# SiTronXD/vk3dGaussianSplatting

Hardware: AMD Instinct MI355X
Metric: Msplats/s + total frame ms (InitSortList/RadixSort/FindRanges/Render split) (higher is better)
Workload: dtype f32; 1 GPU; Garden-30k shape: 5,834,784 gaussians @ 1920x1080; num_gaussians=5834784, width=1920, height=1080, render_mode=exact, render_kernel=auto, sort_algorithm=radix4, frames_in_flight=1, parallelism=single GPU

## Files before the change

### vk3dgaussiansplatting_amd/csrc/gs_project.hip

```cpp
#include <cstdlib>
#include "gs_splat_math.h"
#include "gs_sort_words.h"

namespace gs {

__device__ __forceinline__ Mat3 mat3_mul(const Mat3& a, const Mat3& b) {
    Mat3 c;
#pragma unroll
    for (int j = 0; j < 3; ++j)
#pragma unroll
        for (int i = 0; i < 3; ++i) {
            float acc = a.m[0][i] * b.m[j][0];
            acc = acc + a.m[1][i] * b.m[j][1];
            acc = acc + a.m[2][i] * b.m[j][2];
            c.m[j][i] = acc;
        }
    return c;
}
__device__ __forceinline__ Mat3 mat3_transpose(const Mat3& a) {
    Mat3 t;
#pragma unroll
    for (int j = 0; j < 3; ++j)
#pragma unroll
        for (int i = 0; i < 3; ++i) t.m[j][i] = a.m[i][j];
// ... 284 lines not shown

    if (g < n && !wave_skip) {
        const float px = scene.pos[g], py = scene.pos[(size_t)n + g], pz = scene.pos[2 * (size_t)n + g];
        float vp[4];
        mat4_mul_vec4(fp.view, px, py, pz, 1.0f, vp);
        if (!(-vp[2] <= fp.near_plane)) {
            float q[4];
            mat4_mul_vec4(fp.proj, vp[0], vp[1], vp[2], vp[3], q);
            const float ndc_x = q[0] / q[3];
            const float ndc_y = q[1] / q[3];
            if (!(fabsf(ndc_x) > fp.ndc_cull || fabsf(ndc_y) > fp.ndc_cull)) {
                float nd = (-vp[2] - fp.near_plane) / (fp.far_plane - fp.near_plane);
                nd = clampf(nd, 0.0f, 1.0f);
                const uint32_t depth_key = f2u_sat(nd * 4294967296.0f);
                bool band_skip = false;

                if (band) {
                    const float hgt = (float)fp.height;
                    const float tfx = fp.tan_fov_y * (float)fp.width / hgt;
                    const float tx = clampf(vp[0] / vp[2], -tfx * fp.in_view_limit, tfx * fp.in_view_limit);
                    const float ty = clampf(vp[1] / vp[2], -fp.tan_fov_y * fp.in_view_limit, fp.tan_fov_y * fp.in_view_limit);
                    const float rmax = radius_bound(fp, tx, ty, vp[2], scene.sig2[g]);
                    const float sy_b = (1.0f - ndc_y) * 0.5f * hgt;
                    band_skip = misses_owned_rows(fp, sy_b - rmax, sy_b + rmax);
                }
                if (!band_skip) {
                    float scale[3], rot[4], cov[3], cov0[3];
#pragma unroll
                    for (int a = 0; a < 3; ++a) scale[a] = scene.scale[a * (size_t)n + g];
#pragma unroll
                    for (int a = 0; a < 4; ++a) rot[a] = scene.rot[a * (size_t)n + g];
                    get_covariance(fp, scale, rot, vp, cov, cov0);

                    float sx, sy;
                    screen_position(fp, ndc_x, ndc_y, sx, sy);

                    const float det = cov[0] * cov[2] - cov[1] * cov[1];
                    const float radius = tile_extent_radius(cov[0], cov[1], cov[2]);
                    const int gw = (int)fp.grid_w, gh = (int)fp.grid_h;
                    const int min_x = clampi(f2i_sat((sx - radius) / 16.0f), 0, gw);
                    const int min_y = clampi(f2i_sat((sy - radius) / 16.0f), 0, gh);
                    int tx = f2i_sat((sx + radius) / 16.0f);
                    int ty = f2i_sat((sy + radius) / 16.0f);
                    const int max_x = clampi(tx == 2147483647 ? tx : tx + 1, 0, gw);
                    const int max_y = clampi(ty == 2147483647 ? ty : ty + 1, 0, gh);

                    int y0 = min_y > (int)fp.row_begin ? min_y : (int)fp.row_begin;
                    int y1 = max_y < (int)fp.row_end ? max_y : (int)fp.row_end;
                    if (y1 < y0) y1 = y0;
                    const int k0 = owned_rows_below(fp, y0), k1 = owned_rows_below(fp, y1);
                    count = (uint32_t)(max_x - min_x) * (uint32_t)(k1 - k0);

                    kept = true;
                    rec0 = make_float4(sx, sy, 0.0f, 0.0f);
                    rec2 = make_float4(0.0f, cov[0], cov[1], cov[2]);
                    if (count != 0u) {
                        float opacity = scene.opacity[g];
                        float inv_x = 0.0f, inv_y = 0.0f, inv_z = 0.0f;
                        if (det != 0.0f) {
                            const float det_inv = 1.0f / det;
                            inv_x = cov[2] * det_inv;
                            inv_y = -cov[1] * det_inv;
                            inv_z = cov[0] * det_inv;
                            if constexpr (AA) {
                                const float det0 = cov0[0] * cov0[2] - cov0[1] * cov0[1];
                                const float r = det0 / det;
                                opacity = opacity * sqrtf(r > kAntialiasFloor ? (r < 1.0f ? r : 1.0f) : kAntialiasFloor);
                            }
                        } else {
                            opacity = 0.0f;
                        }
                        rec0.z = inv_x; rec0.w = inv_y;
                        rec2.x = opacity;
                        if constexpr (VIEW_Z) {
                            sc.view_z[g] = -vp[2];
                            sc.depth_key[g] = depth_key;
                            sc.extents[g] = make_uint2((uint32_t)min_x | ((uint32_t)k0 << 16), (uint32_t)max_x | ((uint32_t)k1 << 16));
                        }
                        float res[3];
                        splat_colour<NT_SH, SH_K>(fp, scene.sh + g, n, px, py, pz, res);
                        rec1 = make_float4(inv_z, res[0], res[1], res[2]);
                        if constexpr (!VIEW_Z) sc.depth_key[g] = depth_key;
#if GS_EMIT_PASS0
                        count |= (depth_key & (uint32_t)(kBins - 1)) << 28;
#endif
                        if constexpr (!VIEW_Z) sc.extents[g] = make_uint2((uint32_t)min_x | ((uint32_t)k0 << 16),
                                                                          (uint32_t)max_x | ((uint32_t)k1 << 16));
                    }
                }
            }
        }
#if GS_EMIT_PASS0
        sc.tiles_touched[g] = count & 0x0FFFFFFFu;
#else
        sc.tiles_touched[g] = count;
#endif
    } else if (g < n) {
        sc.tiles_touched[g] = 0u;
    }

#if GS_EMIT_PASS0
    const uint32_t digit = count >> 28;
    count &= 0x0FFFFFFFu;
#endif
    s_raster[threadIdx.x * 3 + 0] = rec0;
    s_raster[threadIdx.x * 3 + 1] = rec1;
    s_raster[threadIdx.x * 3 + 2] = rec2;
    const uint32_t wsum = wave_sum_to_lane63(count);
    const uint64_t emits = __ballot(count != 0u);
    const uint32_t wflags = (uint32_t)__popcll(emits);
    const bool wave_kept = __ballot(kept) != 0ull;
#if GS_EMIT_PASS0
    __shared__ uint32_t s_hist[kProjThreads / 64][kBins];
    if (lane_id() < kBins) s_hist[wave_id()][lane_id()] = 0u;
    __builtin_amdgcn_wave_barrier();
    for (uint64_t todo = emits; todo != 0ull;) {
        const uint32_t d = (uint32_t)__builtin_amdgcn_readlane((int)digit, (int)__builtin_ctzll(todo));
        const bool mine = count != 0u && digit == d;
        const uint32_t dsum = wave_sum_to_lane63(mine ? count : 0u);
        if (lane_id() == 63) s_hist[wave_id()][d] = dsum;
        todo &= ~__ballot(mine);
    }
#endif
    if (lane_id() == 63) {
        s_wave_sum[wave_id()] = wsum;
        s_wave_flags[wave_id()] = wflags;
#ifndef GS_PROJECT_WRITE_ALL
#define GS_PROJECT_WRITE_ALL 0
#endif
#ifndef GS_PROJECT_WRITE_KEPT
#define GS_PROJECT_WRITE_KEPT 0
#endif
#ifndef GS_PROJECT_RECORD_CHUNK
#define GS_PROJECT_RECORD_CHUNK 16
#endif
        static_assert(GS_PROJECT_RECORD_CHUNK == 16 || GS_PROJECT_RECORD_CHUNK == 64, "a quarter wave or a wave");
        uint32_t wrote;
        if (band) wrote = wsum != 0u ? 0xFu : 0u;
        else if (GS_PROJECT_WRITE_ALL || GS_PROJECT_WRITE_KEPT) wrote = (GS_PROJECT_WRITE_ALL || wave_kept) ? 0xFu : 0u;
        else if (GS_PROJECT_RECORD_CHUNK == 64) wrote = emits != 0ull ? 0xFu : 0u;
        else wrote = ((emits & 0xFFFFull) ? 1u : 0u) | ((emits & 0xFFFF0000ull) ? 2u : 0u) |
                     ((emits & 0xFFFF00000000ull) ? 4u : 0u) | ((emits >> 48) ? 8u : 0u);
        s_wave_emits[wave_id()] = wrote;
        sc.wave_wrote[blk * (kProjThreads / 64) + wave_id()] = (uint8_t)wrote;
    }
    __syncthreads();
    {
        const uint32_t first = blk * kProjThreads;
        const uint32_t valid = (n - first) < (uint32_t)kProjThreads ? (n - first) : (uint32_t)kProjThreads;
        float4* out = reinterpret_cast<float4*>(sc.raster + first);
#pragma unroll
        for (int q = 0; q < 3; ++q) {
            const uint32_t i = q * kProjThreads + threadIdx.x;
            if (i < valid * 3u && ((s_wave_emits[i / 192u] >> ((i / 48u) & 3u)) & 1u)) out[i] = s_raster[i];
        }
    }
    uint32_t t = 0;
#pragma unroll
    for (int w = 0; w < kProjThreads / 64; ++w) t += s_wave_sum[w];
    if (threadIdx.x == 0) {
        sc.block_sums[blk] = t;
        if (fp.splat_first) sc.block_flags[blk] = s_wave_flags[0] + s_wave_flags[1] + s_wave_flags[2] + s_wave_flags[3];
    }
#if GS_EMIT_PASS0
    if (threadIdx.x < kBins) {
        const uint32_t v = (s_hist[0][threadIdx.x] + s_hist[1][threadIdx.x]) + (s_hist[2][threadIdx.x] + s_hist[3][threadIdx.x]);
        const uint32_t nb = (n + (uint32_t)kProjThreads - 1u) / (uint32_t)kProjThreads;
        uint32_t* hist = pass0_hist_of(sc.block_sums, nb);
        uint32_t* chunk = pass0_chunk_of(sc.block_sums, nb);
        hist[(size_t)blk * kBins + threadIdx.x] = v;
        if (v != 0u)
            (void)__hip_atomic_fetch_add(&chunk[((size_t)fp.parity * pass0_chunks(nb) + blk / kPass0Chunk) * kBins + threadIdx.x],
                                         v, __ATOMIC_RELAXED, __HIP_MEMORY_SCOPE_AGENT);
    }
#endif
    if (!fp.splat_first) register_emit_helpers(fp, sc, blk, t);
}

struct ScanJob { const uint32_t* sums; uint32_t* offsets; SortParams* params; uint32_t capacity;
                 uint32_t* host_note;
                 SortParams* done_params; };
constexpr uint32_t kScanClearWgs = 8;
struct Pass0Scan { const uint32_t* hist; uint32_t* offs; const uint32_t* chunk_in; uint4* chunk_zero; uint32_t chunks; };

__device__ __forceinline__ void scan_pass0_chunk(const Pass0Scan& p0, uint32_t c, uint32_t num_blocks) {
    __shared__ uint32_t s_part[16][kBins], s_rows[16][kBins];
    const uint32_t tid = threadIdx.x, lane = tid & 63u, wave = tid >> 6, d = tid & 15u;
    const uint32_t row = c * kPass0Chunk + (tid >> 4);
    const uint32_t v = row < num_blocks ? p0.hist[(size_t)row * kBins + d] : 0u;
    uint32_t before = 0u;
    for (uint32_t k = tid >> 4; k < c; k += 64u) before += p0.chunk_in[(size_t)k * kBins + d];
    before += (uint32_t)__shfl_xor((int)before, 16, 64);
    before += (uint32_t)__shfl_xor((int)before, 32, 64);
    uint32_t inc = v;
    uint32_t up = (uint32_t)__shfl_up((int)inc, 16, 64);
    inc += lane >= 16u ? up : 0u;
    up = (uint32_t)__shfl_up((int)inc, 32, 64);
    inc += lane >= 32u ? up : 0u;
    if (lane < (uint32_t)kBins) s_part[wave][d] = before;
    if (lane >= 48u) s_rows[wave][d] = inc;
    __syncthreads();
    uint32_t base = 0u;
#pragma unroll
    for (uint32_t w = 0; w < 16u; ++w) base += s_part[w][d] + (w < wave ? s_rows[w][d] : 0u);
    if (row <= num_blocks) p0.offs[(size_t)row * kBins + d] = base + inc - v;
}

__global__ __launch_bounds__(1024) void k_scan_blocks(const ScanJob job0, const ScanJob job1, uint32_t jobs, uint32_t num_blocks,
                                                       uint4* __restrict__ zero_a, uint32_t n16_a,
                                                       uint4* __restrict__ zero_b, uint32_t n16_b,
                                                       uint32_t* __restrict__ next_help_count, const Pass0Scan p0) {
    if (blockIdx.x >= jobs + kScanClearWgs) {
        scan_pass0_chunk(p0, blockIdx.x - jobs - kScanClearWgs, num_blocks);
        return;
    }
    if (blockIdx.x >= jobs) {
        const uint32_t k = blockIdx.x - jobs;
        if (k == 0u && threadIdx.x == 0 && next_help_count) { next_help_count[0] = 0u; next_help_count[2] = 0u; }
        for (uint32_t i = k * 1024u + threadIdx.x; i < n16_a; i += kScanClearWgs * 1024u) zero_a[i] = make_uint4(0u, 0u, 0u, 0u);
        for (uint32_t i = k * 1024u + threadIdx.x; i < n16_b; i += kScanClearWgs * 1024u) zero_b[i] = make_uint4(0u, 0u, 0u, 0u);
        for (uint32_t i = k * 1024u + threadIdx.x; i < p0.chunks * 4u; i += kScanClearWgs * 1024u) p0.chunk_zero[i] = make_uint4(0u, 0u, 0u, 0u);
        return;
    }
    const ScanJob job = blockIdx.x == 0 ? job0 : job1;
    const uint32_t* __restrict__ block_sums = job.sums;
    uint32_t* __restrict__ block_offsets = job.offsets;
    SortParams* params = job.params;
    const uint32_t capacity = job.capacity;
    __shared__ uint64_t s_wave_tot[16];
    const int tid = threadIdx.x, lane = tid & 63, wave = tid >> 6;
    const uint32_t per = (((num_blocks + 1023u) / 1024u) + 3u) & ~3u;
    const uint4* in4 = reinterpret_cast<const uint4*>(block_sums + (size_t)tid * per);
    uint4* out4 = reinterpret_cast<uint4*>(block_offsets + (size_t)tid * per);
    auto sat = [](uint64_t x) { return (uint32_t)(x > 0xFFFFFFFFull ? 0xFFFFFFFFull : x); };
    constexpr uint32_t kHeld = 8;
    const bool held = per / 4 <= kHeld;
    uint4 v[kHeld];
    uint64_t sum = 0;
    if (held) {
#pragma unroll
        for (uint32_t i = 0; i < kHeld; ++i) v[i] = i < per / 4 ? in4[i] : make_uint4(0u, 0u, 0u, 0u);
#pragma unroll
        for (uint32_t i = 0; i < kHeld; ++i) sum += (uint64_t)v[i].x + v[i].y + v[i].z + v[i].w;
    } else {
#pragma unroll 4
        for (uint32_t i = 0; i < per / 4; ++i) {
            const uint4 w = in4[i];
            sum += (uint64_t)w.x + w.y + w.z + w.w;
        }
    }
    const uint64_t inc = wave_inclusive_scan64(sum);
    if (lane == 63) s_wave_tot[wave] = inc;
    __syncthreads();
    uint64_t run = inc - sum;
    for (int w = 0; w < wave; ++w) run += s_wave_tot[w];
    if (tid == 1023) {
        const uint64_t counter = run + sum;
        const uint32_t e = counter < capacity ? (uint32_t)counter : capacity;
        params->counter = counter;
        params->num_elems = e;
        params->num_groups = (e + kSortTile - 1) / kSortTile;
        params->groups_per_seg = (params->num_groups + kSegments - 1) / kSegments;
        params->overflow = counter > capacity ? 1u : 0u;
        if (job.done_params) {
            const bool redo = counter > capacity;
            job.done_params->counter = counter;
            job.done_params->num_elems = redo ? e : 0u;
            job.done_params->num_groups = redo ? params->num_groups : 0u;
            job.done_params->groups_per_seg = redo ? params->groups_per_seg : 0u;
            job.done_params->overflow = redo ? 1u : 0u;
        }
        if (job.host_note) __hip_atomic_store(job.host_note, e + 1u, __ATOMIC_RELAXED, __HIP_MEMORY_SCOPE_SYSTEM);
    }
    if (held) {
#pragma unroll
        for (uint32_t i = 0; i < kHeld; ++i) {
            uint4 o;
            o.x = sat(run); run += v[i].x;
            o.y = sat(run); run += v[i].y;
            o.z = sat(run); run += v[i].z;
            o.w = sat(run); run += v[i].w;
            if (i < per / 4) out4[i] = o;
        }
    } else {
#pragma unroll 4
        for (uint32_t i = 0; i < per / 4; ++i) {
            const uint4 w = in4[i];
            uint4 o;
            o.x = sat(run); run += w.x;
            o.y = sat(run); run += w.y;
            o.z = sat(run); run += w.z;
            o.w = sat(run); run += w.w;
            out4[i] = o;
        }
    }
}

constexpr int kEmitChunk = 4 * kProjThreads;
static_assert(kEmitSlice % kEmitChunk == 0, "a slice is a whole number of rounds");

#ifndef GS_EMIT_XCD_ORDER
#define GS_EMIT_XCD_ORDER 0
#endif
template <bool SORTED, bool P0 = false>
__global__ __launch_bounds__(kProjThreads) void k_emit(const FrameParams fp, const SplatScratch sc,
                                                        uint32_t* __restrict__ out_lo,
                                                        uint32_t* __restrict__ out_hi,
                                                        uint32_t* __restrict__ out_id, uint32_t num_blocks,
                                                        uint32_t helpers, const uint32_t* __restrict__ sorted_ids,
                                                        const uint32_t* __restrict__ sorted_counts,
                                                        uint32_t* __restrict__ p0_lo = nullptr, uint32_t* __restrict__ p0_hi = nullptr,
                                                        uint32_t* __restrict__ p0_id = nullptr, const SortParams* __restrict__ done = nullptr) {
    static_assert(!(SORTED && P0), "the splat-first list is in depth order already");
    const uint32_t* __restrict__ sums = SORTED ? sc.sorted_sums : sc.block_sums;
    __shared__ __attribute__((aligned(16))) uint32_t s_dig[P0 ? kBins : 1][kProjThreads / 64];
    __shared__ uint32_t s_gofs[P0 ? kBins : 1];
    __shared__ uint32_t s_tot[P0 ? kBins : 1];
    __shared__ uint8_t s_idx[P0 ? kProjThreads : 1];
    __shared__ uint32_t s_incl[kProjThreads];
    __shared__ uint32_t s_wave_tot[kProjThreads / 64];
    __shared__ uint2 s_ext[kProjThreads];
    __shared__ uint32_t s_depth[kProjThreads];
    __shared__ uint32_t s_owner[kEmitChunk];
    __shared__ uint32_t s_wmax[kProjThreads / 64];
    const uint32_t n = SORTED ? sc.aux_params[0].num_elems : fp.num_gaussians;
    const int tid = threadIdx.x;
    uint32_t blk = blockIdx.x - helpers, slice = 0u;
    if (blockIdx.x < helpers) {
        const uint32_t h = blockIdx.x;
        if (h >= sc.help_count[fp.parity]) return;
        const uint2 rec = sc.help_list[h];
        blk = rec.x; slice = rec.y;
        if (blk >= num_blocks || slice == 0u) return;
        const uint32_t first = sc.help_slot[blk];
        if (first == kEmitNoHelp || h - first + 1u != slice) return;
        const uint32_t t = sums[blk];
        if (t <= kEmitSlice || slice > (t - 1u) / kEmitSlice) return;
    } else if constexpr (P0 && GS_EMIT_XCD_ORDER != 0) {
        blk = xcd_group(blk, (num_blocks + 7u) / 8u);
        if (blk >= num_blocks) return;
    }
    const uint32_t g = blk * kProjThreads + tid;
    const uint32_t total = sums[blk];
    if (!owns_every_row(fp) && total == 0) return;
    const uint32_t base = sc.block_offsets[blk];
    const bool alone = slice == 0u && total > kEmitSlice && sc.help_slot[blk] == kEmitNoHelp;
    uint32_t cnt = 0u, my_depth = 0u;
    uint2 my_ext = make_uint2(0u, 0u);
    if (g < n) {
        if constexpr (SORTED) {
            my_depth = sorted_ids[g];
            cnt = fp.hi16 ? (uint32_t)reinterpret_cast<const uint16_t*>(sorted_counts)[g] : sorted_counts[g];
            my_ext = sc.extents[my_depth];
        } else {
            cnt = sc.tiles_touched[g];
            my_ext = sc.extents[g];
            my_depth = sc.depth_key[g];
        }
    }
    bool fused = false;
    uint32_t my_offs = 0u, dstart16 = 0u;
    if constexpr (P0) {
        fused = done->overflow == 0u;
        if (tid < kBins) {
            my_offs = sc.pass0_offs[(size_t)blk * kBins + tid];
            s_tot[tid] = sc.pass0_offs[(size_t)num_blocks * kBins + tid];
        }
    }
    if (total == 0) return;
    if (base >= fp.capacity) return;
    if (P0 && fused) {
        const uint32_t dg = cnt != 0u ? my_depth & (uint32_t)(kBins - 1) : 0u;
        uint32_t m_lo = 0xFFFFFFFFu, m_hi = 0xFFFFFFFFu;
#pragma unroll
        for (int b = 0; b < kRadixBits; ++b) {
            const int32_t sbit = __builtin_amdgcn_sbfe((int32_t)dg, (uint32_t)b, 1u);
            const uint64_t bal = __ballot(sbit != 0);
            m_lo &= ~((uint32_t)bal ^ (uint32_t)sbit);
            m_hi &= ~((uint32_t)(bal >> 32) ^ (uint32_t)sbit);
        }
        const uint64_t same = ((uint64_t)m_hi << 32) | m_lo;
        const uint32_t in_wave = mbcnt(same);
        if (lane_id() < kBins) s_dig[lane_id()][wave_id()] = 0u;
        __builtin_amdgcn_wave_barrier();
        if (in_wave == 0u) s_dig[dg][wave_id()] = (uint32_t)__popcll(same);
        __syncthreads();
        static_assert(kProjThreads / 64 == 4, "one 16-byte LDS read per digit");
        const uint4 c = *reinterpret_cast<const uint4*>(&s_dig[lane_id() & 15][0]);
        const uint32_t tot = c.x + c.y + c.z + c.w;
        dstart16 = row16_inclusive_scan(tot) - tot;
        const uint32_t wb = dstart16 + (wave_id() > 0 ? c.x : 0u) + (wave_id() > 1 ? c.y : 0u) + (wave_id() > 2 ? c.z : 0u);
        const uint32_t slot = (uint32_t)__shfl((int)wb, (int)dg, 64) + in_wave;
        if ((uint32_t)__shfl((int)tot, (int)dg, 64) == (uint32_t)kProjThreads) {
            s_ext[tid] = my_ext;
            s_depth[tid] = my_depth;
            s_idx[tid] = (uint8_t)tid;
        } else {
            s_incl[slot] = cnt;
            s_ext[slot] = my_ext;
            s_depth[slot] = my_depth;
            s_idx[slot] = (uint8_t)tid;
            __syncthreads();
            cnt = s_incl[tid];
        }
    } else {
        s_ext[tid] = my_ext;
        s_depth[tid] = my_depth;
        if constexpr (P0) s_idx[tid] = (uint8_t)tid;
    }
    const uint32_t inc = wave_inclusive_scan(cnt);
    if (lane_id() == 63) s_wave_tot[wave_id()] = inc;
    __syncthreads();
    uint32_t wbase = 0;
    for (int w = 0; w < wave_id(); ++w) wbase += s_wave_tot[w];
    s_incl[tid] = wbase + inc;
    __syncthreads();
    if constexpr (P0) {
        if (tid < kBins) {
            uint32_t gofs = base;
            if (fused) {
                uint32_t smaller = 0u;
                for (int d = 0; d < tid; ++d) smaller += s_tot[d];
                gofs = smaller + my_offs - (dstart16 > 0u ? s_incl[dstart16 - 1u] : 0u);
            }
            s_gofs[tid] = gofs;
        }
        if (fused) { out_lo = p0_lo; out_hi = p0_hi; out_id = p0_id; }
    }

    const uint32_t g0 = blk * kProjThreads;
    const uint32_t my_excl = s_incl[tid] - cnt;
    const uint32_t c_begin = slice * kEmitSlice;
    const uint32_t c_end = alone || total - c_begin < kEmitSlice ? total : c_begin + kEmitSlice;
    for (uint32_t c0 = c_begin; c0 < c_end; c0 += kEmitChunk) {
#pragma unroll
        for (int k = 0; k < kEmitChunk / kProjThreads; ++k) s_owner[k * kProjThreads + tid] = 0u;
        __syncthreads();
        if (cnt != 0u) {
            if (my_excl >= c0) {
                if (my_excl - c0 < (uint32_t)kEmitChunk) s_owner[my_excl - c0] = (uint32_t)tid + 1u;
            } else if (my_excl + cnt > c0) {
                s_owner[0] = (uint32_t)tid + 1u;
            }
        }
        __syncthreads();
        uint4 o = *reinterpret_cast<const uint4*>(&s_owner[4 * tid]);
        o.y = o.y > o.x ? o.y : o.x;
        o.z = o.z > o.y ? o.z : o.y;
        o.w = o.w > o.z ? o.w : o.z;
        const uint32_t winc = wave_inclusive_max(o.w);
        if (lane_id() == 63) s_wmax[wave_id()] = winc;
        uint32_t prev = __shfl_up(winc, 1, 64);
        if (lane_id() == 0) prev = 0u;
        __syncthreads();
        for (int w = 0; w < wave_id(); ++w) prev = prev > s_wmax[w] ? prev : s_wmax[w];
        o.x = o.x > prev ? o.x : prev;
        o.y = o.y > prev ? o.y : prev;
        o.z = o.z > prev ? o.z : prev;
        o.w = o.w > prev ? o.w : prev;
        *reinterpret_cast<uint4*>(&s_owner[4 * tid]) = o;
        __syncthreads();
#pragma unroll
        for (int k = 0; k < kEmitChunk / kProjThreads; ++k) {
            const uint32_t jj = (uint32_t)(k * kProjThreads + tid);
            const uint32_t j = c0 + jj;
            if (j < total) {
                const uint32_t s = s_owner[jj] - 1u;
                const uint32_t excl = s > 0u ? s_incl[s - 1u] : 0u;
                const uint32_t id_local = j - excl;
                const uint2 ext = s_ext[s];
                const uint32_t min_x = ext.x & 0xFFFFu, y0 = ext.x >> 16, max_x = ext.y & 0xFFFFu;
                const uint32_t wdt = max_x - min_x;
                uint32_t ry = (uint32_t)((float)id_local * __builtin_amdgcn_rcpf((float)wdt));
                int32_t rx = (int32_t)(id_local - ry * wdt);
                if (rx < 0) { --ry; rx += (int32_t)wdt; }
                else if ((uint32_t)rx >= wdt) { ++ry; rx -= (int32_t)wdt; }
                const uint32_t tile_key = (y0 + ry) * fp.grid_w + (min_x + (uint32_t)rx);
                const uint64_t out = P0 ? (uint64_t)(s_gofs[s_depth[s] & (uint32_t)(kBins - 1)] + j) : (uint64_t)base + j;
                const uint32_t id = g0 + (P0 ? (uint32_t)s_idx[s] : s);
                if (out < fp.capacity) {
                    if (!SORTED && fp.packed) {
                        out_lo[out] = s_depth[s];
                        out_id[out] = (tile_key << 16) | (id & 0xFFFFu);
                        reinterpret_cast<uint8_t*>(out_hi)[out] = (uint8_t)(id >> 16);
                    } else {
                        if (fp.hi16) reinterpret_cast<uint16_t*>(out_hi)[out] = (uint16_t)tile_key;
                        else out_hi[out] = tile_key;
                        if constexpr (SORTED) out_id[out] = s_depth[s];
                        else { out_lo[out] = s_depth[s]; out_id[out] = id; }
                    }
                }
            }
        }
        __syncthreads();
    }
}

template <int SH_K, bool AA>
static void launch_project_cut(const FrameParams& fp, const SceneBuffers& scene, const SplatScratch& sc, uint32_t blocks, bool nt_sh,
                               hipStream_t stream) {
    if (sc.view_z) {
        if (nt_sh) hipLaunchKernelGGL((k_project<true, true, SH_K, AA>), dim3(blocks), dim3(kProjThreads), 0, stream, fp, scene, sc, blocks);
        else hipLaunchKernelGGL((k_project<false, true, SH_K, AA>), dim3(blocks), dim3(kProjThreads), 0, stream, fp, scene, sc, blocks);
    } else {
        if (nt_sh) hipLaunchKernelGGL((k_project<true, false, SH_K, AA>), dim3(blocks), dim3(kProjThreads), 0, stream, fp, scene, sc, blocks);
        else hipLaunchKernelGGL((k_project<false, false, SH_K, AA>), dim3(blocks), dim3(kProjThreads), 0, stream, fp, scene, sc, blocks);
    }
}

void launch_project(const FrameParams& fp, const SceneBuffers& scene, const SplatScratch& sc,
                    hipStream_t stream) {
    const uint32_t blocks = (fp.num_gaussians + kProjThreads - 1) / kProjThreads;
    if (blocks == 0) return;
    const bool listed = !(fp.row_begin == 0u && fp.row_end == fp.grid_h) && fp.row_stride == 1u;
    if (listed) hipLaunchKernelGGL(k_band_cull, dim3((blocks * 4u + (uint32_t)kCullThreads - 1u) / (uint32_t)kCullThreads), dim3(kCullThreads), 0, stream,
                                   fp, scene, sc, blocks);
#ifndef GS_PROJECT_NT_SH_ABOVE
#define GS_PROJECT_NT_SH_ABOVE ((size_t)256u << 20)
#endif
    const bool nt_sh = (size_t)fp.num_gaussians * 236u > GS_PROJECT_NT_SH_ABOVE;
    const int cut = sh_cut_of_mode(fp.sh_mode);
    if (fp.antialias) {
        switch (cut) {
            case 4: launch_project_cut<4, true>(fp, scene, sc, blocks, nt_sh, stream); break;
            case 9: launch_project_cut<9, true>(fp, scene, sc, blocks, nt_sh, stream); break;
            default: launch_project_cut<0, true>(fp, scene, sc, blocks, nt_sh, stream); break;
        }
    } else {
        switch (cut) {
            case 4: launch_project_cut<4, false>(fp, scene, sc, blocks, nt_sh, stream); break;
            case 9: launch_project_cut<9, false>(fp, scene, sc, blocks, nt_sh, stream); break;
            default: launch_project_cut<0, false>(fp, scene, sc, blocks, nt_sh, stream); break;
        }
    }
}

template <int SH_K>
__global__ __launch_bounds__(256) void k_debug_colour(const FrameParams fp, const SceneBuffers scene, const float4* records, float4* out) {
    const uint32_t n = fp.num_gaussians;
    const uint32_t g = blockIdx.x * 256u + threadIdx.x;
    if (g >= n) return;
    float4 o = make_float4(0.f, 0.f, 0.f, 0.f);
    if (records[2 * (size_t)g].w != 0.0f) {
        float res[3];
        splat_colour<false, SH_K>(fp, scene.sh + g, n, scene.pos[g], scene.pos[(size_t)n + g], scene.pos[2 * (size_t)n + g], res);
        o = make_float4(res[0], res[1], res[2], 1.0f);
    }
    out[g] = o;
}

void launch_debug_colour(const FrameParams& fp, const SceneBuffers& scene, const float* records, float* out_rgba, hipStream_t stream) {
    const uint32_t blocks = (fp.num_gaussians + 255u) / 256u;
    if (!blocks) return;
    float4* out = reinterpret_cast<float4*>(out_rgba);
    const float4* recs = reinterpret_cast<const float4*>(records);
    switch (sh_cut_of_mode(fp.sh_mode)) {
        case 4: hipLaunchKernelGGL(k_debug_colour<4>, dim3(blocks), dim3(256), 0, stream, fp, scene, recs, out); break;
        case 9: hipLaunchKernelGGL(k_debug_colour<9>, dim3(blocks), dim3(256), 0, stream, fp, scene, recs, out); break;
        default: hipLaunchKernelGGL(k_debug_colour<0>, dim3(blocks), dim3(256), 0, stream, fp, scene, recs, out); break;
    }
}

__global__ __launch_bounds__(256) void k_debug_records(const FrameParams fp, const SceneBuffers scene, const SplatScratch sc, float4* out) {
    const uint32_t n = fp.num_gaussians;
    const uint32_t g = blockIdx.x * 256u + threadIdx.x;
    if (g >= n) return;
    float4 o0 = make_float4(0.f, 0.f, 0.f, 0.f), o1 = o0;
    if (sc.tiles_touched[g] == 0u) {
        float vp[4];
        mat4_mul_vec4(fp.view, scene.pos[g], scene.pos[(size_t)n + g], scene.pos[2 * (size_t)n + g], 1.0f, vp);
        if (!(-vp[2] <= fp.near_plane)) {
            float q[4];
            mat4_mul_vec4(fp.proj, vp[0], vp[1], vp[2], vp[3], q);
            const float ndc_x = q[0] / q[3];
            const float ndc_y = q[1] / q[3];
            if (!(fabsf(ndc_x) > fp.ndc_cull || fabsf(ndc_y) > fp.ndc_cull)) {
                float scale[3], rot[4], cov[3], cov0[3];
#pragma unroll
                for (int a = 0; a < 3; ++a) scale[a] = scene.scale[a * (size_t)n + g];
#pragma unroll
                for (int a = 0; a < 4; ++a) rot[a] = scene.rot[a * (size_t)n + g];
                get_covariance(fp, scale, rot, vp, cov, cov0);
                float sx, sy;
                screen_position(fp, ndc_x, ndc_y, sx, sy);
                o0 = make_float4(sx, sy, 0.0f, 1.0f);
                o1 = make_float4(0.0f, cov[0], cov[1], cov[2]);
            }
        }
    }
    out[2 * (size_t)g] = o0;
    out[2 * (size_t)g + 1] = o1;
}

void launch_debug_records(const FrameParams& fp, const SceneBuffers& scene, const SplatScratch& sc, float* out_records, hipStream_t stream) {
    const uint32_t blocks = (fp.num_gaussians + 255u) / 256u;
    if (!blocks) return;
    hipLaunchKernelGGL(k_debug_records, dim3(blocks), dim3(256), 0, stream, fp, scene, sc, reinterpret_cast<float4*>(out_records));
}

void launch_scan_blocks(const FrameParams& fp, const SplatScratch& sc, SortParams* params,
                        uint32_t* ranges, uint32_t* coarse, hipStream_t stream) {
    const uint32_t blocks = (fp.num_gaussians + kProjThreads - 1) / kProjThreads;
    const uint32_t n16_ranges = (fp.grid_w * fp.grid_h * 2u + 3u) / 4u;
    const uint32_t n16_coarse = (uint32_t)(kMaxSortPasses * kBins * kCoarse) / 4u;
    const ScanJob elements{sc.block_sums, sc.block_offsets, params, fp.capacity, sc.elems_note, GS_EMIT_PASS0 ? params + 1 : nullptr};
    const ScanJob splats{sc.block_flags, sc.flag_offsets, sc.aux_params, fp.num_gaussians, nullptr, nullptr};
    const uint32_t jobs = fp.splat_first ? 2u : 1u;
    const uint32_t chunks = GS_EMIT_PASS0 ? pass0_chunks(blocks) : 0u;
    const size_t half = (size_t)chunks * kBins;
    const Pass0Scan p0{sc.pass0_hist, sc.pass0_offs, sc.pass0_chunk + fp.parity * half,
                       reinterpret_cast<uint4*>(sc.pass0_chunk + (fp.parity ^ 1u) * half), chunks};
    hipLaunchKernelGGL(k_scan_blocks, dim3(jobs + kScanClearWgs + chunks), dim3(1024), 0, stream, elements, splats, jobs, blocks,
                       reinterpret_cast<uint4*>(ranges), n16_ranges, reinterpret_cast<uint4*>(coarse), n16_coarse,
                       sc.help_count + (fp.parity ^ 1u), p0);
}

void launch_emit(const FrameParams& fp, const SplatScratch& sc, const SortBuffers& sb, bool pass0,
                 hipStream_t stream) {
    const uint32_t blocks = (fp.num_gaussians + kProjThreads - 1) / kProjThreads;
    if (blocks == 0) return;
    const uint32_t helpers = emit_helpers(fp.capacity);
    if (pass0) {
        const uint32_t owners = GS_EMIT_XCD_ORDER != 0 ? 8u * ((blocks + 7u) / 8u) : blocks;
        hipLaunchKernelGGL((k_emit<false, true>), dim3(helpers + owners), dim3(kProjThreads), 0, stream, fp, sc, sb.lo[0],
                           sb.hi[0], sb.id[0], blocks, helpers, (const uint32_t*)nullptr, (const uint32_t*)nullptr,
                           sb.lo[1], sb.hi[1], sb.id[1], (const SortParams*)(sb.params + 1));
        return;
    }
    hipLaunchKernelGGL((k_emit<false>), dim3(helpers + blocks), dim3(kProjThreads), 0, stream, fp, sc, sb.lo[0],
                       sb.hi[0], sb.id[0], blocks, helpers, (const uint32_t*)nullptr, (const uint32_t*)nullptr);
}

__global__ __launch_bounds__(kProjThreads) void k_splat_list(const FrameParams fp, const SplatScratch sc,
                                                              uint32_t* __restrict__ out_depth, uint32_t* __restrict__ out_count,
                                                              uint32_t* __restrict__ out_id) {
    __shared__ uint32_t s_cnt[kProjThreads / 64], s_flag[kProjThreads / 64];
    const uint32_t blk = blockIdx.x, g = blk * kProjThreads + threadIdx.x;
    if (blk == 0u && threadIdx.x == 0u) sc.help_count[fp.parity] = 0u;
    if (sc.block_sums[blk] == 0u) return;
    const uint32_t cnt = g < fp.num_gaussians ? sc.tiles_touched[g] : 0u;
    const uint32_t dk = cnt != 0u ? sc.depth_key[g] : 0u;
    const uint64_t off0 = sc.block_offsets[blk];
    const uint32_t fpos0 = sc.flag_offsets[blk];
    const uint32_t inc = wave_inclusive_scan(cnt);
    const uint64_t fb = __ballot(cnt != 0u);
    if (lane_id() == 63) { s_cnt[wave_id()] = inc; s_flag[wave_id()] = (uint32_t)__popcll(fb); }
    __syncthreads();
    uint64_t off = off0 + (inc - cnt);
    uint32_t pos = fpos0 + (uint32_t)__popcll(fb & ((1ull << lane_id()) - 1ull));
    for (int w = 0; w < wave_id(); ++w) { off += s_cnt[w]; pos += s_flag[w]; }
    if (cnt != 0u) {
        const uint64_t room = off < fp.capacity ? (uint64_t)fp.capacity - off : 0ull;
        const uint32_t kept = room < cnt ? (uint32_t)room : cnt;
        out_depth[pos] = dk;
        if (fp.hi16) reinterpret_cast<uint16_t*>(out_count)[pos] = (uint16_t)kept;
        else out_count[pos] = kept;
        out_id[pos] = g;
    }
}

constexpr int kSumsBlocksPerWg = 8;
__global__ __launch_bounds__(kProjThreads) void k_sorted_sums(const FrameParams fp, const SplatScratch sc,
                                                               const uint32_t* __restrict__ sorted_counts, uint32_t num_blocks) {
    const uint32_t ve = sc.aux_params[0].num_elems;
    const int lane = lane_id();
#pragma unroll
    for (int it = 0; it < kSumsBlocksPerWg / (kProjThreads / 64); ++it) {
        const uint32_t blk = blockIdx.x * kSumsBlocksPerWg + (uint32_t)(it * (kProjThreads / 64) + wave_id());
        if (blk >= num_blocks) return;
        const uint32_t i0 = blk * kProjThreads + 4u * (uint32_t)lane;
        uint32_t c[4] = {0u, 0u, 0u, 0u};
        if (i0 + 3u < ve) {
            if (fp.hi16) {
                const uint2 v = *reinterpret_cast<const uint2*>(reinterpret_cast<const uint16_t*>(sorted_counts) + i0);
                c[0] = v.x & 0xFFFFu; c[1] = v.x >> 16; c[2] = v.y & 0xFFFFu; c[3] = v.y >> 16;
            } else {
                const uint4 v = *reinterpret_cast<const uint4*>(sorted_counts + i0);
                c[0] = v.x; c[1] = v.y; c[2] = v.z; c[3] = v.w;
            }
        } else {
#pragma unroll
            for (int k = 0; k < 4; ++k)
                if (i0 + k < ve) c[k] = fp.hi16 ? (uint32_t)reinterpret_cast<const uint16_t*>(sorted_counts)[i0 + k] : sorted_counts[i0 + k];
        }
        const uint32_t t = (uint32_t)__builtin_amdgcn_readlane((int)wave_sum_to_lane63(c[0] + c[1] + c[2] + c[3]), 63);
        if (lane == 0) sc.sorted_sums[blk] = t;
        if (t > kEmitSlice) {
            const uint32_t extra = (t - 1u) / kEmitSlice;
            uint32_t slot = 0u;
            if (lane == 0) {
                slot = atomicAdd(&sc.help_count[fp.parity], extra);
                if ((uint64_t)slot + extra > (uint64_t)emit_helpers(fp.capacity)) slot = kEmitNoHelp;
                sc.help_slot[blk] = slot;
            }
            slot = (uint32_t)__builtin_amdgcn_readfirstlane((int)slot);
            if (slot != kEmitNoHelp)
                for (uint32_t i = (uint32_t)lane; i < extra; i += 64u) sc.help_list[slot + i] = make_uint2(blk, i + 1u);
        }
    }
}

void launch_splat_list(const FrameParams& fp, const SplatScratch& sc, const SortBuffers& sb, hipStream_t stream) {
    const uint32_t blocks = (fp.num_gaussians + kProjThreads - 1) / kProjThreads;
    if (blocks == 0) return;
    hipLaunchKernelGGL(k_splat_list, dim3(blocks), dim3(kProjThreads), 0, stream, fp, sc, sb.lo[1], sb.hi[1], sb.id[1]);
}

void launch_gather_sorted(const FrameParams& fp, const SplatScratch& sc, const SortBuffers& sb, int sorted, hipStream_t stream) {
    const uint32_t blocks = (fp.num_gaussians + kProjThreads - 1) / kProjThreads;
    if (blocks == 0) return;
    hipLaunchKernelGGL(k_sorted_sums, dim3((blocks + kSumsBlocksPerWg - 1) / kSumsBlocksPerWg), dim3(kProjThreads), 0, stream, fp, sc,
                       (const uint32_t*)sb.hi[sorted], blocks);
    const ScanJob sorted_blocks{sc.sorted_sums, sc.block_offsets, sc.aux_params + 1, fp.capacity};
    hipLaunchKernelGGL(k_scan_blocks, dim3(1), dim3(1024), 0, stream, sorted_blocks, sorted_blocks, 1u, blocks,
                       (uint4*)nullptr, 0u, (uint4*)nullptr, 0u, (uint32_t*)nullptr, Pass0Scan{});
}

void launch_emit_sorted(const FrameParams& fp, const SplatScratch& sc, const SortBuffers& sb, int sorted, hipStream_t stream) {
    const uint32_t blocks = (fp.num_gaussians + kProjThreads - 1) / kProjThreads;
    if (blocks == 0) return;
    const uint32_t helpers = emit_helpers(fp.capacity);
    hipLaunchKernelGGL((k_emit<true>), dim3(helpers + blocks), dim3(kProjThreads), 0, stream, fp, sc, (uint32_t*)nullptr,
                       sb.hi[0], sb.id[0], blocks, helpers, (const uint32_t*)sb.id[sorted], (const uint32_t*)sb.hi[sorted]);
}

}
```

Baseline: 6613 Msplats/s.

## Add slot-record emit path for fused pass0 with per-splat records in LDS

Adds a dedicated emit kernel body for the fused pass-0 path. It packs each splat's count, extents, index and depth into one LDS record, pre-sorts splats within the block by low depth digit, and computes owners with a vectorized max-scan. Each output element then does a single LDS record read instead of several scattered arrays, and the next block's loads are prefetched when a workgroup handles multiple blocks. The aim is fewer LDS accesses and barriers in the emit stage, at the cost of more code, more LDS use, and extra ballot and scan work per block.

```diff
diff --git a/vk3dgaussiansplatting_amd/csrc/gs_project.hip b/vk3dgaussiansplatting_amd/csrc/gs_project.hip
--- a/vk3dgaussiansplatting_amd/csrc/gs_project.hip
+++ b/vk3dgaussiansplatting_amd/csrc/gs_project.hip
@@ -610,15 +610,15 @@
 #ifndef GS_EMIT_XCD_ORDER
 #define GS_EMIT_XCD_ORDER 0
 #endif
-template <bool SORTED, bool P0 = false>
-__global__ __launch_bounds__(kProjThreads) void k_emit(const FrameParams fp, const SplatScratch sc,
-                                                        uint32_t* __restrict__ out_lo,
-                                                        uint32_t* __restrict__ out_hi,
-                                                        uint32_t* __restrict__ out_id, uint32_t num_blocks,
-                                                        uint32_t helpers, const uint32_t* __restrict__ sorted_ids,
-                                                        const uint32_t* __restrict__ sorted_counts,
-                                                        uint32_t* __restrict__ p0_lo = nullptr, uint32_t* __restrict__ p0_hi = nullptr,
-                                                        uint32_t* __restrict__ p0_id = nullptr, const SortParams* __restrict__ done = nullptr) {
+template <bool SORTED, bool P0>
+__device__ __forceinline__ void emit_walk(const FrameParams& fp, const SplatScratch& sc,
+                                          uint32_t* __restrict__ out_lo,
+                                          uint32_t* __restrict__ out_hi,
+                                          uint32_t* __restrict__ out_id, uint32_t num_blocks,
+                                          uint32_t helpers, const uint32_t* __restrict__ sorted_ids,
+                                          const uint32_t* __restrict__ sorted_counts,
+                                          uint32_t* __restrict__ p0_lo, uint32_t* __restrict__ p0_hi,
+                                          uint32_t* __restrict__ p0_id, const SortParams* __restrict__ done) {
     static_assert(!(SORTED && P0), "the splat-first list is in depth order already");
     const uint32_t* __restrict__ sums = SORTED ? sc.sorted_sums : sc.block_sums;
     __shared__ __attribute__((aligned(16))) uint32_t s_dig[P0 ? kBins : 1][kProjThreads / 64];
@@ -804,6 +804,227 @@
     }
 }
 
+#ifndef GS_EMIT_SLOT_RECORDS
+#define GS_EMIT_SLOT_RECORDS 1
+#endif
+#ifndef GS_EMIT_BLOCKS_PER_WG
+#define GS_EMIT_BLOCKS_PER_WG 1
+#endif
+__host__ __device__ inline uint32_t emit_owner_wgs(uint32_t blocks) {
+    return GS_EMIT_SLOT_RECORDS != 0 ? (blocks + (uint32_t)GS_EMIT_BLOCKS_PER_WG - 1u) / (uint32_t)GS_EMIT_BLOCKS_PER_WG : blocks;
+}
+__device__ __forceinline__ void emit_slots(const FrameParams& fp, const SplatScratch& sc,
+                                           uint32_t* __restrict__ out_lo, uint32_t* __restrict__ out_hi, uint32_t* __restrict__ out_id,
+                                           uint32_t num_blocks, uint32_t helpers,
+                                           uint32_t* __restrict__ p0_lo, uint32_t* __restrict__ p0_hi, uint32_t* __restrict__ p0_id,
+                                           const SortParams* __restrict__ done) {
+    static_assert(kProjThreads / 64 == 4 && kEmitChunk == 4 * kProjThreads, "four waves, four elements per thread and round");
+    __shared__ __attribute__((aligned(16))) uint32_t s_dig[kBins][kProjThreads / 64];
+    __shared__ __attribute__((aligned(16))) uint32_t s_below[kProjThreads / 64][kProjThreads / 64];
+    __shared__ uint32_t s_first[kBins];
+    __shared__ uint32_t s_wave_tot[kProjThreads / 64];
+    __shared__ uint4 s_slot[kProjThreads];
+    __shared__ uint2 s_put[kProjThreads];
+    __shared__ __attribute__((aligned(16))) uint32_t s_owner[kEmitChunk];
+    const uint32_t* __restrict__ sums = sc.block_sums;
+    const uint32_t n = fp.num_gaussians;
+    const int tid = threadIdx.x;
+    uint32_t blk = (blockIdx.x - helpers) * (uint32_t)GS_EMIT_BLOCKS_PER_WG, slice = 0u, todo = (uint32_t)GS_EMIT_BLOCKS_PER_WG;
+    if (blockIdx.x < helpers) {
+        const uint32_t h = blockIdx.x;
+        if (h >= sc.help_count[fp.parity]) return;
+        const uint2 rec = sc.help_list[h];
+        blk = rec.x; slice = rec.y; todo = 1u;
+        if (blk >= num_blocks || slice == 0u) return;
+        const uint32_t first = sc.help_slot[blk];
+        if (first == kEmitNoHelp || h - first + 1u != slice) return;
+        const uint32_t t = sums[blk];
+        if (t <= kEmitSlice || slice > (t - 1u) / kEmitSlice) return;
+    } else {
+        if constexpr (GS_EMIT_XCD_ORDER != 0)
+            blk = xcd_group(blockIdx.x - helpers, (emit_owner_wgs(num_blocks) + 7u) / 8u) * (uint32_t)GS_EMIT_BLOCKS_PER_WG;
+        if (blk >= num_blocks) return;
+        if (num_blocks - blk < todo) todo = num_blocks - blk;
+    }
+    const bool fused = done->overflow == 0u;
+    uint32_t d16 = 0u;
+    {
+        const uint32_t* __restrict__ tot = sc.pass0_offs + (size_t)num_blocks * kBins;
+        uint32_t run = 0u;
+#pragma unroll
+        for (int d = 0; d < kBins; ++d) {
+            d16 = (tid & (kBins - 1)) == d ? run : d16;
+            run += tot[d];
+        }
+    }
+    uint32_t totals[GS_EMIT_BLOCKS_PER_WG], bases[GS_EMIT_BLOCKS_PER_WG];
+#pragma unroll
+    for (uint32_t q = 0; q < (uint32_t)GS_EMIT_BLOCKS_PER_WG; ++q) {
+        const uint32_t b = blk + q < num_blocks ? blk + q : num_blocks - 1u;
+        totals[q] = sums[b];
+        bases[q] = sc.block_offsets[b];
+    }
+    struct Loads { uint32_t cnt, depth, offs16; uint2 ext; };
+    auto load = [&](uint32_t b) {
+        Loads l;
+        const uint32_t g = b * kProjThreads + tid, gc = g < n ? g : n - 1u;
+        l.cnt = sc.tiles_touched[gc];
+        l.ext = sc.extents[gc];
+        l.depth = sc.depth_key[gc];
+        l.offs16 = sc.pass0_offs[(size_t)b * kBins + (tid & (kBins - 1))];
+        return l;
+    };
+    Loads next = load(blk);
+    *reinterpret_cast<uint4*>(&s_owner[4 * tid]) = make_uint4(0u, 0u, 0u, 0u);
+#pragma unroll
+    for (uint32_t q = 0; q < (uint32_t)GS_EMIT_BLOCKS_PER_WG; ++q, ++blk) {
+        if (q >= todo) break;
+        const Loads cur = next;
+        const bool last_block = q + 1u == todo;
+        if (!last_block) next = load(blk + 1u);
+        const uint32_t total = totals[q], base = bases[q];
+        if (total == 0) continue;
+        if (base >= fp.capacity) return;
+        const bool alone = slice == 0u && total > kEmitSlice && sc.help_slot[blk] == kEmitNoHelp;
+        uint32_t cnt = blk * kProjThreads + tid < n ? cur.cnt : 0u, depth = cur.depth;
+        uint2 ext = cur.ext;
+        uint32_t idx = (uint32_t)tid;
+        uint32_t dstart16 = 0u, gbase16 = base;
+        ext.y &= 0xFFFFu;
+        if (fused) {
+            gbase16 = d16 + cur.offs16;
+            const uint32_t dg = cnt != 0u ? depth & (uint32_t)(kBins - 1) : 0u;
+            uint32_t m_lo = 0xFFFFFFFFu, m_hi = 0xFFFFFFFFu;
+#pragma unroll
+            for (int b = 0; b < kRadixBits; ++b) {
+                const int32_t sbit = __builtin_amdgcn_sbfe((int32_t)dg, (uint32_t)b, 1u);
+                const uint64_t bal = __ballot(sbit != 0);
+                m_lo &= ~((uint32_t)bal ^ (uint32_t)sbit);
+                m_hi &= ~((uint32_t)(bal >> 32) ^ (uint32_t)sbit);
+            }
+            const uint64_t same = ((uint64_t)m_hi << 32) | m_lo;
+            const uint32_t in_wave = mbcnt(same);
+            if (lane_id() < kBins) s_dig[lane_id()][wave_id()] = 0u;
+            __builtin_amdgcn_wave_barrier();
+            if (in_wave == 0u) s_dig[dg][wave_id()] = (uint32_t)__popcll(same);
+            __syncthreads();
+            const uint4 c = *reinterpret_cast<const uint4*>(&s_dig[lane_id() & 15][0]);
+            const uint32_t tot = c.x + c.y + c.z + c.w;
+            dstart16 = row16_inclusive_scan(tot) - tot;
+            const uint32_t wb = dstart16 + (wave_id() > 0 ? c.x : 0u) + (wave_id() > 1 ? c.y : 0u) + (wave_id() > 2 ? c.z : 0u);
+            const uint32_t slot = (uint32_t)__shfl((int)wb, (int)dg, 64) + in_wave;
+            if ((uint32_t)__shfl((int)tot, (int)dg, 64) != (uint32_t)kProjThreads) {
+                s_slot[slot] = make_uint4(cnt, ext.x, ext.y | ((uint32_t)tid << 16), depth);
+                __syncthreads();
+                const uint4 r = s_slot[tid];
+                cnt = r.x; ext.x = r.y; ext.y = r.z & 0xFFFFu; idx = r.z >> 16; depth = r.w;
+            }
+        }
+        const uint32_t inc = wave_inclusive_scan(cnt);
+        if (lane_id() == 63) s_wave_tot[wave_id()] = inc;
+        __syncthreads();
+        uint32_t my_excl = inc - cnt;
+        for (int w = 0; w < wave_id(); ++w) my_excl += s_wave_tot[w];
+        s_slot[tid] = make_uint4(my_excl, ext.x, ext.y, depth);
+        const uint32_t dslot = cnt != 0u ? depth & (uint32_t)(kBins - 1) : 0u;
+        const uint32_t gb = (uint32_t)__shfl((int)gbase16, (int)dslot, 64);
+        if (fused) {
+            if ((uint32_t)__shfl((int)dstart16, (int)dslot, 64) == (uint32_t)tid) s_first[dslot] = my_excl;
+            out_lo = p0_lo; out_hi = p0_hi; out_id = p0_id;
+        }
+
+        const uint32_t g0 = blk * kProjThreads;
+        const uint32_t c_begin = slice * kEmitSlice;
+        const uint32_t c_end = alone || total - c_begin < kEmitSlice ? total : c_begin + kEmitSlice;
+        for (uint32_t c0 = c_begin; c0 < c_end; c0 += kEmitChunk) {
+            if (cnt != 0u) {
+                if (my_excl >= c0) {
+                    if (my_excl - c0 < (uint32_t)kEmitChunk) s_owner[my_excl - c0] = (uint32_t)tid + 1u;
+                } else if (my_excl + cnt > c0) {
+                    s_owner[0] = (uint32_t)tid + 1u;
+                }
+            }
+#pragma unroll
+            for (uint32_t k = 1; k < (uint32_t)(kProjThreads / 64); ++k) {
+                const uint64_t bal = __ballot(cnt != 0u && my_excl < c0 + k * (uint32_t)kProjThreads);
+                if (lane_id() == 0)
+                    s_below[k][wave_id()] = bal != 0ull ? (uint32_t)(wave_id() * 64 + 64 - __builtin_clzll(bal)) : 0u;
+            }
+            __syncthreads();
+            if (c0 == c_begin) s_put[tid] = make_uint2(fused ? gb - s_first[dslot] : base, g0 + idx);
+            uint4 o = *reinterpret_cast<const uint4*>(&s_owner[4 * tid]);
+            o.y = o.y > o.x ? o.y : o.x;
+            o.z = o.z > o.y ? o.z : o.y;
+            o.w = o.w > o.z ? o.w : o.z;
+            const uint32_t winc = wave_inclusive_max(o.w);
+            uint32_t prev = __shfl_up(winc, 1, 64);
+            if (lane_id() == 0) prev = 0u;
+            if (wave_id() > 0) {
+                const uint4 b = *reinterpret_cast<const uint4*>(&s_below[wave_id()][0]);
+                const uint32_t b01 = b.x > b.y ? b.x : b.y, b23 = b.z > b.w ? b.z : b.w;
+                const uint32_t bm = b01 > b23 ? b01 : b23;
+                prev = prev > bm ? prev : bm;
+            }
+            o.x = o.x > prev ? o.x : prev;
+            o.y = o.y > prev ? o.y : prev;
+            o.z = o.z > prev ? o.z : prev;
+            o.w = o.w > prev ? o.w : prev;
+            *reinterpret_cast<uint4*>(&s_owner[4 * tid]) = o;
+            __syncthreads();
+            const bool more = c0 + (uint32_t)kEmitChunk < c_end || !last_block;
+            asm volatile("" : "+v"(next.cnt), "+v"(next.depth), "+v"(next.offs16), "+v"(next.ext.x), "+v"(next.ext.y));
+#pragma unroll
+            for (int k = 0; k < kEmitChunk / kProjThreads; ++k) {
+                const uint32_t jj = (uint32_t)(k * kProjThreads + tid);
+                const uint32_t j = c0 + jj;
+                const uint32_t s = s_owner[jj] - 1u;
+                if (more) s_owner[jj] = 0u;
+                if (j < total) {
+                    const uint4 r = s_slot[s];
+                    const uint2 put = s_put[s];
+                    const uint32_t id_local = j - r.x;
+                    const uint32_t min_x = r.y & 0xFFFFu, y0 = r.y >> 16;
+                    const uint32_t wdt = r.z - min_x;
+                    uint32_t ry = (uint32_t)((float)id_local * __builtin_amdgcn_rcpf((float)wdt));
+                    int32_t rx = (int32_t)(id_local - ry * wdt);
+                    if (rx < 0) { --ry; rx += (int32_t)wdt; }
+                    else if ((uint32_t)rx >= wdt) { ++ry; rx -= (int32_t)wdt; }
+                    const uint32_t tile_key = (y0 + ry) * fp.grid_w + (min_x + (uint32_t)rx);
+                    const uint64_t out = (uint64_t)(put.x + j);
+                    if (out < fp.capacity) {
+                        if (fp.packed) {
+                            out_lo[out] = r.w;
+                            out_id[out] = (tile_key << 16) | (put.y & 0xFFFFu);
+                            reinterpret_cast<uint8_t*>(out_hi)[out] = (uint8_t)(put.y >> 16);
+                        } else {
+                            if (fp.hi16) reinterpret_cast<uint16_t*>(out_hi)[out] = (uint16_t)tile_key;
+                            else out_hi[out] = tile_key;
+                            out_lo[out] = r.w;
+                            out_id[out] = put.y;
+                        }
+                    }
+                }
+            }
+            if (more) __syncthreads();
+        }
+    }
+}
+
+template <bool SORTED, bool P0 = false>
+__global__ __launch_bounds__(kProjThreads) void k_emit(const FrameParams fp, const SplatScratch sc,
+                                                        uint32_t* __restrict__ out_lo,
+                                                        uint32_t* __restrict__ out_hi,
+                                                        uint32_t* __restrict__ out_id, uint32_t num_blocks,
+                                                        uint32_t helpers, const uint32_t* __restrict__ sorted_ids,
+                                                        const uint32_t* __restrict__ sorted_counts,
+                                                        uint32_t* __restrict__ p0_lo = nullptr, uint32_t* __restrict__ p0_hi = nullptr,
+                                                        uint32_t* __restrict__ p0_id = nullptr, const SortParams* __restrict__ done = nullptr) {
+    if constexpr (P0 && GS_EMIT_SLOT_RECORDS != 0)
+        emit_slots(fp, sc, out_lo, out_hi, out_id, num_blocks, helpers, p0_lo, p0_hi, p0_id, done);
+    else
+        emit_walk<SORTED, P0>(fp, sc, out_lo, out_hi, out_id, num_blocks, helpers, sorted_ids, sorted_counts, p0_lo, p0_hi, p0_id, done);
+}
+
 template <int SH_K, bool AA>
 static void launch_project_cut(const FrameParams& fp, const SceneBuffers& scene, const SplatScratch& sc, uint32_t blocks, bool nt_sh,
                                hipStream_t stream) {
@@ -929,7 +1150,8 @@
     if (blocks == 0) return;
     const uint32_t helpers = emit_helpers(fp.capacity);
     if (pass0) {
-        const uint32_t owners = GS_EMIT_XCD_ORDER != 0 ? 8u * ((blocks + 7u) / 8u) : blocks;
+        const uint32_t wgs = emit_owner_wgs(blocks);
+        const uint32_t owners = GS_EMIT_XCD_ORDER != 0 ? 8u * ((wgs + 7u) / 8u) : wgs;
         hipLaunchKernelGGL((k_emit<false, true>), dim3(helpers + owners), dim3(kProjThreads), 0, stream, fp, sc, sb.lo[0],
                            sb.hi[0], sb.id[0], blocks, helpers, (const uint32_t*)nullptr, (const uint32_t*)nullptr,
                            sb.lo[1], sb.hi[1], sb.id[1], (const SortParams*)(sb.params + 1));
```

Result: no change. 6636 Msplats/s (median of 6 runs) (+0.4%).
